# ShioMisaka/fce-yolo

Measured on AMD Instinct MI355X. Metric: images/sec/GPU @ 640x640 bs=32, yolo11n-fce; fraction of fp16 MFMA roofline, higher is better.
Workload: dtype fp16; 1 GPU; yolo11n-fce detection inference (forward + decode + NMS) @ 640x640, 32 images/GPU; model=yolo11n-fce, global_batch=32, imgsz=640, parallelism=dp1, batches_in_flight=4, distinct_inputs=5, hw_queues=8, forward_launch=hipgraph

## Files before the change

### fce-yolo_amd/csrc/stem_fused.hip

```cpp
#include <algorithm>
#include <type_traits>

#include "mfma_stage.h"
#include "ops.h"

namespace fce {

struct Stem2Args {
  const void* x;
  int N, H, W;
  int Hs, Ws;
  int Ho, Wo;
  const h8* w0;
  const float* b0;
  const h8* w1;
  int nalloc1;
  const float* b1;
  _Float16* y;
  int ycs;
};

template <int C0, int C1, int SR2>
struct StG {
  static constexpr int IR = 4 * SR2 + 3;
  static constexpr int NS = 2 * SR2 + 1;
  static constexpr int K1 = C0 / 8, sS = K1 | 1;
  static constexpr int RC0 = C0 / 16, CT1 = C1 / 16;
  static constexpr bool CM = C0 % 32 == 0;
  static constexpr int NS1 = CM ? 9 * (C0 / 32) : (9 * K1 + 3) / 4;
  static_assert(C0 % 16 == 0 && C1 % 16 == 0, "stem fused: channel configuration");
};

template <typename T>
struct StRaw {
  h8 v;
  __device__ __forceinline__ void load(const T* p) { v = *reinterpret_cast<const h8*>(p); }
  __device__ __forceinline__ void zero() { v = h8{0, 0, 0, 0, 0, 0, 0, 0}; }
  __device__ __forceinline__ h8 half8() const { return v; }
};
template <>
struct StRaw<float> {
  f4 a, b;
  __device__ __forceinline__ void load(const float* p) {
    a = reinterpret_cast<const f4*>(p)[0];
    b = reinterpret_cast<const f4*>(p)[1];
  }
  __device__ __forceinline__ void zero() { a = b = f4{0.f, 0.f, 0.f, 0.f}; }
  __device__ __forceinline__ h8 half8() const {
    return h8{(_Float16)a[0], (_Float16)a[1], (_Float16)a[2], (_Float16)a[3],
              (_Float16)b[0], (_Float16)b[1], (_Float16)b[2], (_Float16)b[3]};
  }
};
template <>
struct StRaw<uint8_t> {
  uint2 v;
  __device__ __forceinline__ void load(const uint8_t* p) { v = *reinterpret_cast<const uint2*>(p); }
  __device__ __forceinline__ void zero() { v = uint2{0u, 0u}; }
  __device__ __forceinline__ h8 half8() const {
    h8 o;
#pragma unroll
    for (int j = 0; j < 8; ++j) {
      const unsigned u = ((j < 4 ? v.x : v.y) >> ((j & 3) * 8)) & 255u;
      o[j] = (_Float16)(float)(_Float16)((float)u / 255.0f);
    }
    return o;
  }
};

template <typename T, int C0, int C1, int SR2, int NW, int NXE>
__global__ __launch_bounds__(NW * 64, 1) void stem_fused_kernel(Stem2Args a) {
  using G = StG<C0, C1, SR2>;
  constexpr int NT = NW * 64;
  extern __shared__ __attribute__((aligned(16))) _Float16 ssm[];
  const int lane = threadIdx.x & 63, wave = threadIdx.x >> 6, col = lane & 15, grp = lane >> 4;
  const int tid = threadIdx.x;
  const int rows = (a.Ho + SR2 - 1) / SR2, ngroups = a.N * rows;
  const int NG = gridDim.x, bi = blockIdx.x;
  const int g_begin = int(int64_t(bi) * ngroups / NG), g_end = int(int64_t(bi + 1) * ngroups / NG);
  if (g_begin >= g_end) return;
  const int WP = a.W + 16, CW = WP / 8;
  const int npos = a.Ws + 2, half = (npos + 1) / 2;
  _Float16* IN = ssm;
  h8* S = reinterpret_cast<h8*>(ssm + 3 * G::IR * WP);
  const int ne = 3 * G::IR * CW;
  const T* x = static_cast<const T*>(a.x);
  StRaw<T> xr[NXE];
  auto load_in = [&](int g) {
    const int n = g / rows, iy0 = 4 * (g - n * rows) * SR2 - 3;
#pragma unroll
    for (int k = 0; k < NXE; ++k) {
      const int e = tid + k * NT;
      const int cr = e / CW, q = e - cr * CW;
      const int ci = cr / G::IR, r = cr - ci * G::IR;
      const int iy = iy0 + r, ix0 = (q - 1) * 8;
      if (e < ne && iy >= 0 && iy < a.H && q >= 1 && ix0 < a.W)
        xr[k].load(x + ((int64_t(n) * 3 + ci) * a.H + iy) * a.W + ix0);
      else
        xr[k].zero();
    }
  };
  load_in(g_begin);
  int koff[8];
#pragma unroll
  for (int j = 0; j < 8; ++j) {
    const int kq = 8 * grp + j, ci = kq / 9, t = kq - ci * 9;
    koff[j] = kq < 27 ? (ci * G::IR + t / 3) * WP + (t % 3) : 0;
  }
  h8 af[G::RC0];
  float bz0[G::RC0][4];
#pragma unroll
  for (int r = 0; r < G::RC0; ++r) {
    af[r] = a.w0[r * 64 + lane];
#pragma unroll
    for (int j = 0; j < 4; ++j) bz0[r][j] = a.b0[r * 16 + grp * 4 + j];
  }
  h8 a1[G::CT1][G::NS1];
  float bz1[G::CT1][4];
#pragma unroll
  for (int ct = 0; ct < G::CT1; ++ct) {
#pragma unroll
    for (int st = 0; st < G::NS1; ++st) a1[ct][st] = a.w1[(size_t(ct) * a.nalloc1 + st) * 64 + lane];
#pragma unroll
    for (int j = 0; j < 4; ++j) bz1[ct][j] = a.b1[ct * 16 + grp * 4 + j];
  }
  const int fps = (a.Ws + 15) / 16, fpo = (a.Wo + 15) / 16;
  constexpr int FMAX = (SR2 * 10 + NW - 1) / NW;
  for (int g = g_begin; g < g_end; ++g) {
    const int n = g / rows, oy0 = (g - n * rows) * SR2;
    const uint32_t yimg = uint32_t(a.Ho) * uint32_t(a.Wo) * uint32_t(a.ycs);
    const __amdgpu_buffer_rsrc_t yr = out_rsrc(a.y + int64_t(n) * yimg, yimg * 2u);
    const int sy0 = 2 * oy0 - 1;
#pragma unroll
    for (int k = 0; k < NXE; ++k) {
      const int e = tid + k * NT;
      if (e < ne) {
        const int cr = e / CW, q = e - cr * CW;
        *reinterpret_cast<h8*>(IN + cr * WP + q * 8) = xr[k].half8();
      }
    }
    if (g + 1 < g_end) load_in(g + 1);
    stage_barrier();
    for (int rr = 0; rr < G::NS; ++rr) {
      const int sy = sy0 + rr;
      h8* Srow = S + rr * npos * G::sS;
      if (sy < 0 || sy >= a.Hs) {
        for (int e = tid; e < npos * G::K1; e += NT) Srow[(e / G::K1) * G::sS + e % G::K1] = h8{0, 0, 0, 0, 0, 0, 0, 0};
        continue;
      }
      if (tid < 2 * G::K1) {
        const int c = tid / G::K1 ? a.Ws + 1 : 0;
        const int p = (c & 1) ? half + (c >> 1) : (c >> 1);
        Srow[p * G::sS + tid % G::K1] = h8{0, 0, 0, 0, 0, 0, 0, 0};
      }
      for (int fx = wave; fx < fps; fx += NW) {
        const int ox = fx * 16 + col;
        const int base = (2 * rr) * WP + 2 * min(ox, a.Ws - 1) + 7;
        h8 b;
#pragma unroll
        for (int j = 0; j < 8; ++j) b[j] = IN[base + koff[j]];
        const int c = ox + 1, p = (c & 1) ? half + (c >> 1) : (c >> 1);
        _Float16* so = reinterpret_cast<_Float16*>(Srow + p * G::sS);
#pragma unroll
        for (int r = 0; r < G::RC0; ++r) {
          const f4 d = __builtin_amdgcn_mfma_f32_16x16x32_f16(af[r], b, f4{0.f, 0.f, 0.f, 0.f}, 0, 0, 0);
          if (ox < a.Ws) {
            h4 o;
#pragma unroll
            for (int j = 0; j < 4; ++j) {
              const float t = d[j] + bz0[r][j];
              o[j] = (_Float16)silu(t);
            }
            *reinterpret_cast<h4*>(so + r * 16 + grp * 4) = o;
          }
        }
      }
    }
    stage_barrier();
#pragma unroll
    for (int i = 0; i < FMAX; ++i) {
      const int f = wave + NW * i;
      const int r1 = f / fpo, fx = f - r1 * fpo;
      const int oy = oy0 + r1;
      const bool wv = f < SR2 * fpo && oy < a.Ho;
      const int ox = fx * 16 + col, oxc = min(ox, a.Wo - 1);
      f4 acc[G::CT1];
#pragma unroll
      for (int ct = 0; ct < G::CT1; ++ct) acc[ct] = f4{0.f, 0.f, 0.f, 0.f};
      if (wv) {
#pragma unroll
        for (int st = 0; st < G::NS1; ++st) {
          int tap, cc;
          bool ok;
          if (G::CM) {
            tap = st % 9;
            cc = (st / 9) * 4 + grp;
            ok = true;
          } else {
            const int c = st * 4 + grp;
            tap = c / G::K1;
            cc = c - tap * G::K1;
            ok = c < 9 * G::K1;
          }
          h8 b = h8{0, 0, 0, 0, 0, 0, 0, 0};
          if (ok) {
            const int ky = tap / 3, kx = tap - ky * 3;
            const int cp = 2 * oxc + kx, p = (cp & 1) ? half + (cp >> 1) : (cp >> 1);
            b = S[((2 * r1 + ky) * npos + p) * G::sS + cc];
          }
#pragma unroll
          for (int ct = 0; ct < G::CT1; ++ct) acc[ct] = __builtin_amdgcn_mfma_f32_16x16x32_f16(a1[ct][st], b, acc[ct], 0, 0, 0);
        }
      }
      const bool ok = wv && ox < a.Wo;
      const uint32_t off = uint32_t((oy * a.Wo + ox) * a.ycs + grp * 4) * 2u;
#pragma unroll
      for (int ct = 0; ct < G::CT1; ++ct) {
        float v[4];
#pragma unroll
        for (int j = 0; j < 4; ++j) v[j] = silu(acc[ct][j] + bz1[ct][j]);
        store_h4_or_drop(yr, ok, off + uint32_t(ct * 32), h4_of(v));
      }
    }
    stage_barrier();
  }
}

static constexpr int kStemInsts[][2] = {{16, 32}, {32, 64}};

bool stem_fused_ok(const fce_stem2_desc& d) {
  for (const auto& s : kStemInsts)
    if (s[0] == d.c0 && s[1] == d.c1) return true;
  return false;
}

bool stem_fused_fits(const fce_stem2_desc& d, int h, int w) { return stem_fused_ok(d) && h > 0 && w % 8 == 0 && w <= 640; }

template <typename T, int C0, int C1, int SR2, int NW>
static int st_launch(const Stem2Args& a, hipStream_t s) {
  using G = StG<C0, C1, SR2>;
  constexpr int NXE_MAX = (3 * G::IR * (640 + 16) / 8 + NW * 64 - 1) / (NW * 64);
  const int ne = 3 * G::IR * (a.W + 16) / 8;
  FCE_CHECK(ne <= NXE_MAX * NW * 64, "stem fused: input wider than the prefetch register image (W <= 640)");
  FCE_CHECK((a.Wo + 15) / 16 <= 10, "stem fused: output wider than the per-wave fragment count (W <= 640)");
  const size_t lds = size_t(3) * G::IR * (a.W + 16) * sizeof(_Float16) + size_t(G::NS) * (a.Ws + 2) * G::sS * 16;
  FCE_CHECK(lds <= 160 * 1024, "stem fused: input too wide for the LDS tile");
  auto k = stem_fused_kernel<T, C0, C1, SR2, NW, NXE_MAX>;
  static const bool big = hipFuncSetAttribute(reinterpret_cast<const void*>(k),
                                              hipFuncAttributeMaxDynamicSharedMemorySize, 160 * 1024) == hipSuccess;
  if (!big && lds > 64 * 1024) return fail(FCE_ERR_HIP, "stem fused: cannot opt in to >64 KiB LDS");
  const int64_t groups = int64_t(a.N) * ((a.Ho + SR2 - 1) / SR2);
  FCE_CHECK(groups > 0 && groups < (int64_t(1) << 31), "stem fused: grid size");
  static int cus = 0;
  if (!cus) {
    int dev = 0;
    if (hipGetDevice(&dev) != hipSuccess || hipDeviceGetAttribute(&cus, hipDeviceAttributeMultiprocessorCount, dev) != hipSuccess)
      cus = 256;
  }
  int occ = 0;
  if (hipOccupancyMaxActiveBlocksPerMultiprocessor(&occ, k, NW * 64, lds) != hipSuccess || occ < 1) occ = 1;
  const int grid = int(std::min<int64_t>(groups, int64_t(cus) * occ));
  FCE_LAUNCH(k, dim3(unsigned(grid)), dim3(NW * 64), lds, s, a);
  return launch_status("stem_fused_kernel");
}

template <typename T>
static int st_dispatch(const Stem2Args& a, int c0, hipStream_t s) {
  const char* e = getenv("FCE_STEM2_SR");
  const char* w = getenv("FCE_STEM2_NW");
  const int sr = e && *e ? atoi(e) : (c0 == 16 ? 2 : 1), nw = w && *w ? atoi(w) : (c0 == 16 ? 8 : 4);
  if (c0 == 16) {
    if (sr == 1 && nw == 4) return st_launch<T, 16, 32, 1, 4>(a, s);
    if (sr == 1 && nw == 8) return st_launch<T, 16, 32, 1, 8>(a, s);
    if (sr == 2 && nw == 4) return st_launch<T, 16, 32, 2, 4>(a, s);
    if (sr == 2 && nw == 8) return st_launch<T, 16, 32, 2, 8>(a, s);
  } else {
    if (sr == 1 && nw == 4) return st_launch<T, 32, 64, 1, 4>(a, s);
    if (sr == 1 && nw == 8) return st_launch<T, 32, 64, 1, 8>(a, s);
  }
  return fail(FCE_ERR_INVALID, "FCE_STEM2_SR / FCE_STEM2_NW: 1 or 2 rows (1 for c0 32), 4 or 8 waves");
}

int stem_fused(const fce_stem2_desc& d, const fce_tensor& x, const fce_tensor& y, hipStream_t s) {
  FCE_CHECK(stem_fused_ok(d), "stem fused: unsupported channel configuration");
  FCE_CHECK(x.layout == FCE_NCHW && x.c == 3 && x.coff == 0 && x.cstride == 3, "stem fused: dense NCHW 3-channel input");
  FCE_CHECK(x.w % 8 == 0 && x.w <= 640, "stem fused: input width a multiple of 8, at most 640");
  FCE_CHECK(y.layout == FCE_NHWC && y.dtype == FCE_F16 && y.c == d.c1 && y.cstride % 4 == 0 && y.coff % 4 == 0,
            "stem fused: NHWC f16 output view");
  Stem2Args a{};
  a.x = x.data;
  a.N = x.n;
  a.H = x.h;
  a.W = x.w;
  a.Hs = (x.h - 1) / 2 + 1;
  a.Ws = (x.w - 1) / 2 + 1;
  a.Ho = (a.Hs - 1) / 2 + 1;
  a.Wo = (a.Ws - 1) / 2 + 1;
  FCE_CHECK(y.n == x.n && y.h == a.Ho && y.w == a.Wo, "stem fused: output size mismatch");
  a.w0 = reinterpret_cast<const h8*>(static_cast<const char*>(d.w[0]) + size_t(3) * 9 * d.c0 * sizeof(float));
  a.b0 = d.b[0];
  a.w1 = static_cast<const h8*>(d.w[1]);
  a.nalloc1 = stage_nalloc(d.c0, 3);
  a.b1 = d.b[1];
  a.y = static_cast<_Float16*>(y.data) + y.coff;
  a.ycs = y.cstride;
  if (x.dtype == FCE_F16) return st_dispatch<_Float16>(a, d.c0, s);
  if (x.dtype == FCE_F32) return st_dispatch<float>(a, d.c0, s);
  if (x.dtype == FCE_U8) return st_dispatch<uint8_t>(a, d.c0, s);
  return fail(FCE_ERR_INVALID, "stem fused: input dtype");
}

}
```

Measured before the change: 39230 images/sec.

## Reuse halo input and stem rows across consecutive row groups via ring buffers

Turns the LDS input tile and the stem-output rows into ring buffers. When a block processes consecutive row groups of the same image, it reuses the 3 overlapping input rows and the first stem row instead of reloading and recomputing them, and it drops the trailing barrier. The prefetch register image is split into halo and new-row parts, and row indexing gains modular wraparound. It also adds an env-gated clock-diagnostic printf and a grid override, which add some register and branch overhead.

```diff
diff --git a/fce-yolo_amd/csrc/stem_fused.hip b/fce-yolo_amd/csrc/stem_fused.hip
--- a/fce-yolo_amd/csrc/stem_fused.hip
+++ b/fce-yolo_amd/csrc/stem_fused.hip
@@ -18,6 +18,7 @@
   const float* b1;
   _Float16* y;
   int ycs;
+  int diag;
 };
 
 template <int C0, int C1, int SR2>
@@ -67,12 +68,12 @@
   }
 };
 
-template <typename T, int C0, int C1, int SR2, int NW, int NXE>
+template <typename T, int C0, int C1, int SR2, int NW, int NXH, int NXN>
 __global__ __launch_bounds__(NW * 64, 1) void stem_fused_kernel(Stem2Args a) {
   using G = StG<C0, C1, SR2>;
   constexpr int NT = NW * 64;
   extern __shared__ __attribute__((aligned(16))) _Float16 ssm[];
-  const int lane = threadIdx.x & 63, wave = threadIdx.x >> 6, col = lane & 15, grp = lane >> 4;
+  const int lane = threadIdx.x & 63, wave = __builtin_amdgcn_readfirstlane(threadIdx.x >> 6), col = lane & 15, grp = lane >> 4;
   const int tid = threadIdx.x;
   const int rows = (a.Ho + SR2 - 1) / SR2, ngroups = a.N * rows;
   const int NG = gridDim.x, bi = blockIdx.x;
@@ -82,29 +83,47 @@
   const int npos = a.Ws + 2, half = (npos + 1) / 2;
   _Float16* IN = ssm;
   h8* S = reinterpret_cast<h8*>(ssm + 3 * G::IR * WP);
-  const int ne = 3 * G::IR * CW;
   const T* x = static_cast<const T*>(a.x);
-  StRaw<T> xr[NXE];
-  auto load_in = [&](int g) {
+  StRaw<T> xh[NXH], xr[NXN];
+  auto load_rows = [&](auto& xs, int r0, int nr, int g) {
+    constexpr int NX = int(sizeof(xs) / sizeof(xs[0]));
     const int n = g / rows, iy0 = 4 * (g - n * rows) * SR2 - 3;
-#pragma unroll
-    for (int k = 0; k < NXE; ++k) {
+    const int ne = nr * 3 * CW;
+#pragma unroll
+    for (int k = 0; k < NX; ++k) {
       const int e = tid + k * NT;
-      const int cr = e / CW, q = e - cr * CW;
-      const int ci = cr / G::IR, r = cr - ci * G::IR;
-      const int iy = iy0 + r, ix0 = (q - 1) * 8;
+      const int rc = e / CW, q = e - rc * CW;
+      const int r = rc / 3, ci = rc - r * 3;
+      const int iy = iy0 + r0 + r, ix0 = (q - 1) * 8;
       if (e < ne && iy >= 0 && iy < a.H && q >= 1 && ix0 < a.W)
-        xr[k].load(x + ((int64_t(n) * 3 + ci) * a.H + iy) * a.W + ix0);
+        xs[k].load(x + ((int64_t(n) * 3 + ci) * a.H + iy) * a.W + ix0);
       else
-        xr[k].zero();
+        xs[k].zero();
     }
   };
-  load_in(g_begin);
-  int koff[8];
+  auto store_rows = [&](auto& xs, int r0, int nr, int is0) {
+    constexpr int NX = int(sizeof(xs) / sizeof(xs[0]));
+    const int ne = nr * 3 * CW;
+#pragma unroll
+    for (int k = 0; k < NX; ++k) {
+      const int e = tid + k * NT;
+      if (e < ne) {
+        const int rc = e / CW, q = e - rc * CW;
+        const int r = rc / 3, ci = rc - r * 3;
+        int sl = is0 + r0 + r;
+        sl -= sl >= G::IR ? G::IR : 0;
+        *reinterpret_cast<h8*>(IN + (ci * G::IR + sl) * WP + q * 8) = xs[k].half8();
+      }
+    }
+  };
+  load_rows(xh, 0, 3, g_begin);
+  load_rows(xr, 3, 4 * SR2, g_begin);
+  int kst[8], kky[8];
 #pragma unroll
   for (int j = 0; j < 8; ++j) {
     const int kq = 8 * grp + j, ci = kq / 9, t = kq - ci * 9;
-    koff[j] = kq < 27 ? (ci * G::IR + t / 3) * WP + (t % 3) : 0;
+    kst[j] = kq < 27 ? (ci * G::IR + t / 3) * WP + (t % 3) : 0;
+    kky[j] = kq < 27 ? t / 3 : 0;
   }
   h8 af[G::RC0];
   float bz0[G::RC0][4];
@@ -125,24 +144,35 @@
   }
   const int fps = (a.Ws + 15) / 16, fpo = (a.Wo + 15) / 16;
   constexpr int FMAX = (SR2 * 10 + NW - 1) / NW;
+  uint64_t clk[5] = {0, 0, 0, 0, 0}, tprev = a.diag ? __builtin_amdgcn_s_memtime() : 0;
+  auto tick = [&](int k) {
+    if (a.diag) {
+      const uint64_t tn = __builtin_amdgcn_s_memtime();
+      clk[k] += tn - tprev;
+      tprev = tn;
+    }
+  };
   for (int g = g_begin; g < g_end; ++g) {
-    const int n = g / rows, oy0 = (g - n * rows) * SR2;
+    const int n = g / rows, og = g - n * rows, oy0 = og * SR2;
     const uint32_t yimg = uint32_t(a.Ho) * uint32_t(a.Wo) * uint32_t(a.ycs);
     const __amdgpu_buffer_rsrc_t yr = out_rsrc(a.y + int64_t(n) * yimg, yimg * 2u);
     const int sy0 = 2 * oy0 - 1;
-#pragma unroll
-    for (int k = 0; k < NXE; ++k) {
-      const int e = tid + k * NT;
-      if (e < ne) {
-        const int cr = e / CW, q = e - cr * CW;
-        *reinterpret_cast<h8*>(IN + cr * WP + q * 8) = xr[k].half8();
-      }
-    }
-    if (g + 1 < g_end) load_in(g + 1);
+    const bool carry = g != g_begin && og != 0;
+    const int is0 = (4 * oy0) % G::IR, ss0 = (2 * oy0) % G::NS;
+    if (!carry) store_rows(xh, 0, 3, is0);
+    store_rows(xr, 3, 4 * SR2, is0);
+    tick(0);
+    if (g + 1 < g_end) {
+      if (og + 1 == rows) load_rows(xh, 0, 3, g + 1);
+      load_rows(xr, 3, 4 * SR2, g + 1);
+    }
     stage_barrier();
-    for (int rr = 0; rr < G::NS; ++rr) {
+    tick(1);
+    for (int rr = carry ? 1 : 0; rr < G::NS; ++rr) {
       const int sy = sy0 + rr;
-      h8* Srow = S + rr * npos * G::sS;
+      int sl = ss0 + rr;
+      sl -= sl >= G::NS ? G::NS : 0;
+      h8* Srow = S + sl * npos * G::sS;
       if (sy < 0 || sy >= a.Hs) {
         for (int e = tid; e < npos * G::K1; e += NT) Srow[(e / G::K1) * G::sS + e % G::K1] = h8{0, 0, 0, 0, 0, 0, 0, 0};
         continue;
@@ -152,9 +182,19 @@
         const int p = (c & 1) ? half + (c >> 1) : (c >> 1);
         Srow[p * G::sS + tid % G::K1] = h8{0, 0, 0, 0, 0, 0, 0, 0};
       }
+      int il0 = is0 + 2 * rr;
+      il0 -= il0 >= G::IR ? G::IR : 0;
+      int koff[8];
+#pragma unroll
+      for (int j = 0; j < 8; ++j) koff[j] = kst[j];
+      if (il0 + 2 >= G::IR) {
+#pragma unroll
+        for (int j = 0; j < 8; ++j) koff[j] -= il0 + kky[j] >= G::IR ? G::IR * WP : 0;
+      }
+      const int rbase = il0 * WP + 7;
       for (int fx = wave; fx < fps; fx += NW) {
         const int ox = fx * 16 + col;
-        const int base = (2 * rr) * WP + 2 * min(ox, a.Ws - 1) + 7;
+        const int base = rbase + 2 * min(ox, a.Ws - 1);
         h8 b;
 #pragma unroll
         for (int j = 0; j < 8; ++j) b[j] = IN[base + koff[j]];
@@ -175,12 +215,19 @@
         }
       }
     }
+    tick(2);
     stage_barrier();
+    tick(3);
 #pragma unroll
     for (int i = 0; i < FMAX; ++i) {
       const int f = wave + NW * i;
-      const int r1 = f / fpo, fx = f - r1 * fpo;
+      int r1 = 0;
+#pragma unroll
+      for (int k = 1; k < SR2; ++k) r1 += f >= k * fpo;
+      const int fx = f - r1 * fpo;
       const int oy = oy0 + r1;
+      int s1 = ss0 + 2 * r1;
+      s1 -= s1 >= G::NS ? G::NS : 0;
       const bool wv = f < SR2 * fpo && oy < a.Ho;
       const int ox = fx * 16 + col, oxc = min(ox, a.Wo - 1);
       f4 acc[G::CT1];
@@ -190,22 +237,26 @@
 #pragma unroll
         for (int st = 0; st < G::NS1; ++st) {
           int tap, cc;
-          bool ok;
+          bool ok, kyu;
           if (G::CM) {
             tap = st % 9;
             cc = (st / 9) * 4 + grp;
             ok = true;
+            kyu = true;
           } else {
             const int c = st * 4 + grp;
             tap = c / G::K1;
             cc = c - tap * G::K1;
             ok = c < 9 * G::K1;
+            kyu = (st * 4 / G::K1) / 3 == std::min((st * 4 + 3) / G::K1, 8) / 3;
           }
           h8 b = h8{0, 0, 0, 0, 0, 0, 0, 0};
           if (ok) {
             const int ky = tap / 3, kx = tap - ky * 3;
             const int cp = 2 * oxc + kx, p = (cp & 1) ? half + (cp >> 1) : (cp >> 1);
-            b = S[((2 * r1 + ky) * npos + p) * G::sS + cc];
+            int sl = s1 + (kyu ? (G::CM ? st % 9 : st * 4 / G::K1) / 3 : ky);
+            sl -= sl >= G::NS ? G::NS : 0;
+            b = S[(sl * npos + p) * G::sS + cc];
           }
 #pragma unroll
           for (int ct = 0; ct < G::CT1; ++ct) acc[ct] = __builtin_amdgcn_mfma_f32_16x16x32_f16(a1[ct][st], b, acc[ct], 0, 0, 0);
@@ -221,7 +272,14 @@
         store_h4_or_drop(yr, ok, off + uint32_t(ct * 32), h4_of(v));
       }
     }
-    stage_barrier();
+    tick(4);
+  }
+  if (a.diag && blockIdx.x == 0 && threadIdx.x == 0) {
+    const unsigned long long ng = (unsigned long long)(g_end - g_begin);
+    printf("stem fused diag <%d,%d,%d,%d>: %llu groups, clocks per group: x->lds %llu, x-issue+barrier %llu, stem %llu, "
+           "barrier %llu, conv2 %llu\n", C0, C1, SR2, NW, ng, (unsigned long long)clk[0] / ng,
+           (unsigned long long)clk[1] / ng, (unsigned long long)clk[2] / ng, (unsigned long long)clk[3] / ng,
+           (unsigned long long)clk[4] / ng);
   }
 }
 
@@ -238,13 +296,15 @@
 template <typename T, int C0, int C1, int SR2, int NW>
 static int st_launch(const Stem2Args& a, hipStream_t s) {
   using G = StG<C0, C1, SR2>;
-  constexpr int NXE_MAX = (3 * G::IR * (640 + 16) / 8 + NW * 64 - 1) / (NW * 64);
-  const int ne = 3 * G::IR * (a.W + 16) / 8;
-  FCE_CHECK(ne <= NXE_MAX * NW * 64, "stem fused: input wider than the prefetch register image (W <= 640)");
+  constexpr int NXH = (3 * 3 * (640 + 16) / 8 + NW * 64 - 1) / (NW * 64);
+  constexpr int NXN = (3 * 4 * SR2 * (640 + 16) / 8 + NW * 64 - 1) / (NW * 64);
+  const int cw = (a.W + 16) / 8;
+  FCE_CHECK(9 * cw <= NXH * NW * 64 && 12 * SR2 * cw <= NXN * NW * 64,
+            "stem fused: input wider than the prefetch register image (W <= 640)");
   FCE_CHECK((a.Wo + 15) / 16 <= 10, "stem fused: output wider than the per-wave fragment count (W <= 640)");
   const size_t lds = size_t(3) * G::IR * (a.W + 16) * sizeof(_Float16) + size_t(G::NS) * (a.Ws + 2) * G::sS * 16;
   FCE_CHECK(lds <= 160 * 1024, "stem fused: input too wide for the LDS tile");
-  auto k = stem_fused_kernel<T, C0, C1, SR2, NW, NXE_MAX>;
+  auto k = stem_fused_kernel<T, C0, C1, SR2, NW, NXH, NXN>;
   static const bool big = hipFuncSetAttribute(reinterpret_cast<const void*>(k),
                                               hipFuncAttributeMaxDynamicSharedMemorySize, 160 * 1024) == hipSuccess;
   if (!big && lds > 64 * 1024) return fail(FCE_ERR_HIP, "stem fused: cannot opt in to >64 KiB LDS");
@@ -258,7 +318,9 @@
   }
   int occ = 0;
   if (hipOccupancyMaxActiveBlocksPerMultiprocessor(&occ, k, NW * 64, lds) != hipSuccess || occ < 1) occ = 1;
-  const int grid = int(std::min<int64_t>(groups, int64_t(cus) * occ));
+  int grid = int(std::min<int64_t>(groups, int64_t(cus) * occ));
+  const char* ge = getenv("FCE_STEM2_GRID");
+  if (ge && atoi(ge) > 0) grid = std::min(grid, atoi(ge));
   FCE_LAUNCH(k, dim3(unsigned(grid)), dim3(NW * 64), lds, s, a);
   return launch_status("stem_fused_kernel");
 }
@@ -303,6 +365,8 @@
   a.b1 = d.b[1];
   a.y = static_cast<_Float16*>(y.data) + y.coff;
   a.ycs = y.cstride;
+  const char* de = getenv("FCE_STEM2_DIAG");
+  a.diag = de && atoi(de) != 0;
   if (x.dtype == FCE_F16) return st_dispatch<_Float16>(a, d.c0, s);
   if (x.dtype == FCE_F32) return st_dispatch<float>(a, d.c0, s);
   if (x.dtype == FCE_U8) return st_dispatch<uint8_t>(a, d.c0, s);
```

Measured after the change: 39080 images/sec. No clear change (-0.4%).
